# byungsook/deep-fluids

Hardware: AMD Instinct MI355X
Metric: velocity-field voxels/sec (3D 64x96x64 train step), whole job; per-GPU in `per_gpu` (higher is better)
Workload: dtype f32; 1 GPU; cfg3: 3D smoke3 64x96x64 (Z,Y,X) fp32, GeneratorBE3 filters=128 num_conv=4, per-GPU batch 16, full train step (fwd+curl3+jacobian3+L1 losses+bwd+Adam); global_batch=16, batch_per_gpu=16, params=7483523, parallelism=dp1

## Files before the change

### deep_fluids_amd/csrc/conv_wgrad.hip

```cpp
#include "df_common.hpp"

namespace {

using df::ceil_div;
typedef float f32x16 __attribute__((ext_vector_type(16)));
typedef float f32x2 __attribute__((ext_vector_type(2)));
typedef float f32x4 __attribute__((ext_vector_type(4)));

constexpr int kThreads = 256;
constexpr int kMaxRanges = 256;
constexpr int kZeroBytes = 512;
inline int64_t zero_row_bytes(int64_t W, int64_t Cin, int64_t Cout) {
  const int64_t Wp = ceil_div(W, 8) * 8 + 8;
  return Wp * (Cin > 2 * Cout ? Cin : 2 * Cout) * 4 + 64;
}
constexpr int kSmallStreams = 2048;

#ifdef DF_TUNING
int g_wgrad_dbg = 0;
#endif

struct WgradArgs {
  const float* x;
  const float* g;
// ... 1094 lines not shown
#pragma unroll
  for (int i = 0; i < 6; ++i) load_pos(cur, i, i);
  xc[0] = xcomb(0);

  auto tile = [&](int u, int x, const Row& lr, int lpos) {
    __builtin_amdgcn_sched_barrier(0);
    xc[(u + 1) & 7] = xcomb((u + 1) & 7);
    xc[(u + 2) & 7] = xcomb((u + 2) & 7);
    const f32x2 g0 = gcomb(u), g1 = gcomb((u + 1) & 7);
    f32x2 dm = xc[(u + 7) & 7], d0 = xc[u], d1 = xc[(u + 1) & 7], d2 = xc[(u + 2) & 7];
    if (x == 0) dm = f32x2{0.f, 0.f};
    if (x == Wc - 2) d2 = f32x2{0.f, 0.f};
    const f32x2 v0 = (DBG & 4) ? dm : wpk_sub(dm, d1), v1 = (DBG & 4) ? d0 : wpk_add(d0, d1), v2 = (DBG & 4) ? d1 : wpk_sub(d1, d0),
                v3 = (DBG & 4) ? d2 : wpk_sub(d0, d2);
    const f32x2 m1 = (DBG & 4) ? g0 : wpk_add(g0, g1), m2 = (DBG & 4) ? g1 : wpk_sub(g0, g1);
    if (!(DBG & 4)) bsum = wpk_add(bsum, m1);
    __builtin_amdgcn_sched_barrier(0);
    load_pos(lr, (u + 6) & 7, lpos);
    load_pos(lr, (u + 7) & 7, lpos + 1);
    if (UP) {
#pragma unroll
      for (int q = 0; q < 4; ++q) xr[q >> 1][q & 1][(u + 7) & 7] = xr[q >> 1][q & 1][(u + 6) & 7];
    }
    __builtin_amdgcn_sched_barrier(0);
#pragma unroll
    for (int s = 0; s < 2; ++s)
#pragma unroll
      for (int t = 0; t < 2; ++t) {
        acc[0][s][t] = __builtin_amdgcn_mfma_f32_32x32x2f32(v0[s], g0[t], acc[0][s][t], 0, 0, 0);
        acc[1][s][t] = __builtin_amdgcn_mfma_f32_32x32x2f32(v1[s], m1[t], acc[1][s][t], 0, 0, 0);
        if (!UP) acc[2][s][t] = __builtin_amdgcn_mfma_f32_32x32x2f32(v2[s], m2[t], acc[2][s][t], 0, 0, 0);
        acc[3][s][t] = __builtin_amdgcn_mfma_f32_32x32x2f32(v3[s], g1[t], acc[3][s][t], 0, 0, 0);
      }
  };

  for (int pair = p0; pair < p1; pair += pstep) {
    const Row nxt = row_setup(pair + pstep);
#pragma unroll
    for (int x0 = 0; x0 < Wc - 8; x0 += 8) {
#pragma unroll
      for (int u = 0; u < 8; u += 2) tile(u, x0 + u, cur, x0 + u + 6);
    }
    {
      constexpr int x0 = Wc - 8;
      tile(0, x0, cur, x0 + 6);
#pragma unroll
      for (int u = 2; u < 8; u += 2) tile(u, x0 + u, nxt, u - 2);
    }
    cur = nxt;
  }

  if constexpr (CS == 64) {
    float (*sR)[64 * 64] = reinterpret_cast<float (*)[64 * 64]>(lds);
    float (*sBs)[64] = reinterpret_cast<float (*)[64]>(lds + 4 * 64 * 64);
    float* P1 = a.partial + static_cast<int64_t>(range) * 64 * a.Cinp * a.Coutp;
#pragma unroll
    for (int d = 0; d < 4; ++d) {
      if (UP && d == 2) continue;
      const int slot = zy * 4 + d;
#pragma unroll
      for (int s = 0; s < 2; ++s)
#pragma unroll
        for (int t = 0; t < 2; ++t)
#pragma unroll
          for (int e = 0; e < 16; ++e) {
            const int i = (e & 3) + 8 * (e >> 2) + 4 * half;
            sR[sub][(2 * i + s) * 64 + 2 * r + t] = acc[d][s][t][e];
          }
      __syncthreads();
#pragma unroll
      for (int q = 0; q < 16; ++q) {
        const int j = q * kThreads + tid;
        const float v = ((sR[0][j] + sR[1][j]) + sR[2][j]) + sR[3][j];
        P1[(static_cast<int64_t>(slot) * a.Cinp + ci0 + (j >> 6)) * a.Coutp + co0 + (j & 63)] = v;
      }
      __syncthreads();
    }
    if (a.want_bias && GZ && GY && sel == 0 && blockIdx.y == 0) {
      bsum[0] += __shfl_xor(bsum[0], 32, 64);
      bsum[1] += __shfl_xor(bsum[1], 32, 64);
      if (half == 0) { sBs[sub][2 * r] = bsum[0]; sBs[sub][2 * r + 1] = bsum[1]; }
      __syncthreads();
      if (tid < 64) a.bpartial[static_cast<int64_t>(range) * a.Coutp + co0 + tid] = ((sBs[0][tid] + sBs[1][tid]) + sBs[2][tid]) + sBs[3][tid];
    }
    return;
  }
  float* P = a.partial + static_cast<int64_t>(erange) * 64 * a.Cinp * a.Coutp;
#pragma unroll
  for (int d = 0; d < 4; ++d) {
    if (UP && d == 2) continue;
    const int slot = zy * 4 + d;
#pragma unroll
    for (int s = 0; s < 2; ++s)
#pragma unroll
      for (int t = 0; t < 2; ++t)
#pragma unroll
        for (int e = 0; e < 16; ++e) {
          const int i = (e & 3) + 8 * (e >> 2) + 4 * half;
          const int ci = ci0 + 2 * i + s, co = co0 + 2 * r + t;
          P[(static_cast<int64_t>(slot) * a.Cinp + ci) * a.Coutp + co] = acc[d][s][t][e];
        }
  }
  if (do_bias) {
    bsum[0] += __shfl_xor(bsum[0], 32, 64);
    bsum[1] += __shfl_xor(bsum[1], 32, 64);
    if (half == 0) {
      float* pb = a.bpartial + static_cast<int64_t>(erange) * a.Coutp + co0 + 2 * r;
      pb[0] = bsum[0]; pb[1] = bsum[1];
    }
  }
}

template <int WP8, int CS, bool GZ, bool GY, bool UP = false, int DBG = 0>
__global__ __launch_bounds__(kThreads, 1) void wgrad_wxyz_kernel(const WxyzArgs aa) {
  constexpr int NT = ((UP && GZ) ? 1 : 2) * ((UP && GY) ? 1 : 2);
  __shared__ float sLds[CS == 64 ? kWxyzLds : 1];
  const int wg = wxyz_wg(aa.w.nranges * NT);
  wgrad_wxyz_body<WP8, CS, GZ, GY, UP, DBG>(aa, wg / NT, wg % NT, sLds);
}

template <int WP8, int CS, int DBG = 0>
__global__ __launch_bounds__(kThreads, 1) void wgrad_wxyz_fused_kernel(const WxyzArgs aa) {
  const int wg = wxyz_wg(aa.w.nranges * 16);
  const int range = wg >> 4, type = wg & 15;
  const int xiz = type >> 2, xiy = type & 3;
  const bool gz = xiz == 1 || xiz == 2, gy = xiy == 1 || xiy == 2;
  const int sel = (gz ? xiz - 1 : xiz / 3) * 2 + (gy ? xiy - 1 : xiy / 3);
  __shared__ float sLds[CS == 64 ? kWxyzLds : 1];
  if (gz && gy) wgrad_wxyz_body<WP8, CS, true, true, false, DBG>(aa, range, sel, sLds);
  else if (gz) wgrad_wxyz_body<WP8, CS, true, false, false, DBG>(aa, range, sel, sLds);
  else if (gy) wgrad_wxyz_body<WP8, CS, false, true, false, DBG>(aa, range, sel, sLds);
  else wgrad_wxyz_body<WP8, CS, false, false, false, DBG>(aa, range, sel, sLds);
}

template <int WP8, int CS>
__global__ __launch_bounds__(kThreads, 1) void wgrad_wxyz_up_fused_kernel(const WxyzArgs aa) {
  const int wg = wxyz_wg(aa.w.nranges * 9);
  const int range = wg / 9, t9 = wg % 9;
  const int zi = t9 / 3, yi = t9 % 3;
  const bool gz = zi == 1, gy = yi == 1;
  const int selz = zi == 2 ? 1 : 0, sely = yi == 2 ? 1 : 0;
  __shared__ float sLds[CS == 64 ? kWxyzLds : 1];
  if (gz && gy) wgrad_wxyz_body<WP8, CS, true, true, true, 0>(aa, range, 0, sLds);
  else if (gz) wgrad_wxyz_body<WP8, CS, true, false, true, 0>(aa, range, sely, sLds);
  else if (gy) wgrad_wxyz_body<WP8, CS, false, true, true, 0>(aa, range, selz, sLds);
  else wgrad_wxyz_body<WP8, CS, false, false, true, 0>(aa, range, selz * 2 + sely, sLds);
}

constexpr int kStgPos = 2 * 256;
template <int WP8> struct WxyzStage {
  static constexpr int Wc = WP8 * 8, NU = Wc / 4, BI = NU / 4, L = BI + 2;
  static constexpr int kLdsBytes = Wc * kStgPos * 4;
  static_assert(L >= BI + 1 && L <= NU - BI && L + 2 <= NU, "staging ring: write lead outside the barrier window");
  static_assert(kLdsBytes <= 160 * 1024, "staged (x,y,z) weight gradient: LDS image above gfx950's 160 KB");
};
static_assert(kWxyzLds * 4 <= 160 * 1024, "64-channel (x,y,z) weight gradient: LDS above gfx950's 160 KB");

template <int WP8, bool GZ, bool GY>
__device__ __forceinline__ void wgrad_wxyz_staged_body(const WxyzArgs& aa, int range, int sel, float* lds) {
  using ST = WxyzStage<WP8>;
  constexpr int Wc = ST::Wc, NU = ST::NU, BI = ST::BI, L = ST::L;
  const WgradArgs& a = aa.w;
  const int tid = threadIdx.x;
  const int lane = tid & 63;
  const int wave = __builtin_amdgcn_readfirstlane(tid >> 6);
  const int qi = wave >> 1, qj = wave & 1;
  const int half = lane >> 5, r = lane & 31;

  const int xiz = GZ ? 1 + sel / 2 : 3 * (sel / 2);
  const int xiy = GY ? 1 + sel % 2 : 3 * (sel % 2);
  const int zy = xiz * 4 + xiy;
  const int ci0 = qi * 64, co0 = qj * 64;
  const int p0 = range * a.pairs_per_range;
  int p1 = (range + 1) * a.pairs_per_range;
  if (p1 > a.npairs) p1 = a.npairs;

  const float* zb = a.zeros;
  const int yoa = xiy == 0 ? -1 : xiy == 2 ? 1 : 0, yob = xiy == 0 ? 1 : xiy == 1 ? 1 : xiy == 2 ? 0 : 2;
  const int zoa = xiz == 0 ? -1 : xiz == 2 ? 1 : 0, zob = xiz == 0 ? 1 : xiz == 1 ? 1 : xiz == 2 ? 0 : 2;
  const float syf = xiy == 1 ? 1.f : -1.f, szf = xiz == 1 ? 1.f : -1.f;
  const int gya = xiy == 3 ? 1 : 0, gza = xiz == 3 ? 1 : 0;
  const f32x2 sy2 = {syf, syf}, sz2 = {szf, szf};
  const int soff = wave * 128 + 4 * r;
  struct Row { const float* x[2][2]; const float* g[2][2]; };
  auto row_setup = [&](int pair) -> Row {
    Row rw;
    const int trow = 2 * pair + half;
    const bool ok = pair < p1 && trow < aa.ntrows;
    const int yt = trow % aa.Ht;
    const int t = trow / aa.Ht;
    const int zt = t % aa.Dt;
    const int b = t / aa.Dt;
    const int z0 = 2 * zt, y0 = 2 * yt;
    const int64_t bbase = static_cast<int64_t>(b) * a.D;
#pragma unroll
    for (int pz = 0; pz < 2; ++pz) {
      const int zs = z0 + (pz ? zob : zoa);
      const bool zv = ok && zs >= 0 && zs < a.D;
#pragma unroll
      for (int py = 0; py < 2; ++py) {
        const int ys = y0 + (py ? yob : yoa);
        rw.x[pz][py] = (zv && ys >= 0 && ys < a.H) ? a.x + ((bbase + zs) * a.H + ys) * Wc * 128 + soff : zb;
      }
      const int gz = z0 + (pz ? 1 : gza);
#pragma unroll
      for (int py = 0; py < 2; ++py) {
        const int gy = y0 + (py ? 1 : gya);
        const bool need = (pz == 0 || GZ) && (py == 0 || GY);
        rw.g[pz][py] = (need && ok) ? a.g + ((bbase + gz) * a.H + gy) * Wc * 128 + soff : zb;
      }
    }
    return rw;
  };
  auto ld4 = [&](const float* base, int unit) -> f32x4 { return *reinterpret_cast<const f32x4*>(base + unit * (4 * 128)); };
  auto pkfma = [&](f32x2 x, f32x2 y, f32x2 z) -> f32x2 {
    f32x2 d;
    asm("v_pk_fma_f32 %0, %1, %2, %3" : "=v"(d) : "v"(x), "v"(y), "v"(z));
    return d;
  };
  auto fma4 = [&](f32x4 x, f32x2 s, f32x4 z) -> f32x4 {
    const f32x2 lo = pkfma(f32x2{x[0], x[1]}, s, f32x2{z[0], z[1]}), hi = pkfma(f32x2{x[2], x[3]}, s, f32x2{z[2], z[3]});
    return f32x4{lo[0], lo[1], hi[0], hi[1]};
  };

  f32x16 acc[4][2][2];
#pragma unroll
  for (int d = 0; d < 4; ++d)
#pragma unroll
    for (int s = 0; s < 2; ++s)
#pragma unroll
      for (int t = 0; t < 2; ++t)
#pragma unroll
        for (int e = 0; e < 16; ++e) acc[d][s][t][e] = 0.f;
  f32x2 bsum = {0.f, 0.f};
  const bool do_bias = a.want_bias && GZ && GY && sel == 0 && qi == 0;

  f32x4 sx[2][2][2], sg[2][2][2];
  float* const wst = lds + wave * kStgPos + half * 256 + 4 * r;
  const float* const rdx = lds + half * 256 + ci0 + 2 * r;
  const float* const rdg = lds + half * 256 + 128 + co0 + 2 * r;
  auto load_x = [&](const Row& lr, int set, int unit) {
#pragma unroll
    for (int q = 0; q < 4; ++q) sx[set][q >> 1][q & 1] = ld4(lr.x[q >> 1][q & 1], unit);
  };
  auto load_g = [&](const Row& lr, int set, int unit) {
    sg[set][0][0] = ld4(lr.g[0][0], unit);
    if (GY) sg[set][0][1] = ld4(lr.g[0][1], unit);
    if (GZ) sg[set][1][0] = ld4(lr.g[1][0], unit);
    if (GZ && GY) sg[set][1][1] = ld4(lr.g[1][1], unit);
  };
  auto store_x = [&](int set, int unit) {
    const f32x4 ta = fma4(sx[set][0][1], sy2, sx[set][0][0]), tb = fma4(sx[set][1][1], sy2, sx[set][1][0]);
    *reinterpret_cast<f32x4*>(wst + unit * (4 * kStgPos)) = fma4(tb, sz2, ta);
  };
  auto store_g = [&](int set, int unit) {
    f32x4 v;
    if (GZ && GY) {
      const f32x4 ta = fma4(sg[set][0][1], sy2, sg[set][0][0]), tb = fma4(sg[set][1][1], sy2, sg[set][1][0]);
      v = fma4(tb, sz2, ta);
    } else if (GY) v = fma4(sg[set][0][1], sy2, sg[set][0][0]);
    else if (GZ) v = fma4(sg[set][1][0], sz2, sg[set][0][0]);
    else v = sg[set][0][0];
    *reinterpret_cast<f32x4*>(wst + unit * (4 * kStgPos) + 128) = v;
  };
  auto lds_sync = [&]() { asm volatile("s_waitcnt lgkmcnt(0)\n\ts_barrier" ::: "memory"); };

  f32x2 xq[8], gq[4];
  auto rd_x = [&](int pos) { xq[pos & 7] = *reinterpret_cast<const f32x2*>(rdx + (pos % Wc) * kStgPos); };
  auto rd_g = [&](int pos) { gq[pos & 3] = *reinterpret_cast<const f32x2*>(rdg + (pos % Wc) * kStgPos); };

  Row cur = row_setup(p0);
#pragma unroll
  for (int u = 0; u < L; ++u) {
    load_x(cur, u & 1, u); load_g(cur, u & 1, u);
    store_x(u & 1, u); store_g(u & 1, u);
  }
#pragma unroll
  for (int u = L; u < L + 2; ++u) { load_x(cur, u & 1, u); load_g(cur, u & 1, u); }
  lds_sync();
  rd_x(0); rd_x(1); rd_x(2); rd_g(0); rd_g(1);
  xq[7] = f32x2{0.f, 0.f};

  auto step = [&](int u, const Row& lc, const Row& ln) {
    const int x = 2 * u, k = u >> 1;
    __builtin_amdgcn_sched_barrier(0);
    const f32x2 g0 = gq[x & 3], g1 = gq[(x + 1) & 3];
    f32x2 dm = xq[(x + 7) & 7], d0 = xq[x & 7], d1 = xq[(x + 1) & 7], d2 = xq[(x + 2) & 7];
    if (x == 0) dm = f32x2{0.f, 0.f};
    if (x == Wc - 2) d2 = f32x2{0.f, 0.f};
    const f32x2 v0 = wpk_sub(dm, d1), v1 = wpk_add(d0, d1), v2 = wpk_sub(d1, d0), v3 = wpk_sub(d0, d2);
    const f32x2 m1 = wpk_add(g0, g1), m2 = wpk_sub(g0, g1);
    bsum = wpk_add(bsum, m1);
    __builtin_amdgcn_sched_barrier(0);
    rd_x(x + 3); rd_x(x + 4); rd_g(x + 2); rd_g(x + 3);
    {
      const int m = k + L, set = m & 1;
      if ((u & 1) == 0) {
        store_x(set, m % NU);
        load_x(m + 2 < NU ? lc : ln, set, (m + 2) % NU);
      } else {
        store_g(set, m % NU);
        load_g(m + 2 < NU ? lc : ln, set, (m + 2) % NU);
      }
    }
    __builtin_amdgcn_sched_barrier(0);
#pragma unroll
    for (int s = 0; s < 2; ++s)
#pragma unroll
      for (int t = 0; t < 2; ++t) {
        acc[0][s][t] = __builtin_amdgcn_mfma_f32_32x32x2f32(v0[s], g0[t], acc[0][s][t], 0, 0, 0);
        acc[1][s][t] = __builtin_amdgcn_mfma_f32_32x32x2f32(v1[s], m1[t], acc[1][s][t], 0, 0, 0);
        acc[2][s][t] = __builtin_amdgcn_mfma_f32_32x32x2f32(v2[s], m2[t], acc[2][s][t], 0, 0, 0);
        acc[3][s][t] = __builtin_amdgcn_mfma_f32_32x32x2f32(v3[s], g1[t], acc[3][s][t], 0, 0, 0);
      }
    if ((u & 1) && (k + 1) % BI == 0) lds_sync();
  };

  for (int pair = p0; pair < p1; ++pair) {
    const Row nxt = row_setup(pair + 1);
#pragma unroll
    for (int u = 0; u < Wc / 2; ++u) step(u, cur, nxt);
    cur = nxt;
  }

  float* P = a.partial + static_cast<int64_t>(range) * 64 * a.Cinp * a.Coutp;
#pragma unroll
  for (int d = 0; d < 4; ++d) {
    const int slot = zy * 4 + d;
#pragma unroll
    for (int s = 0; s < 2; ++s)
#pragma unroll
      for (int t = 0; t < 2; ++t)
#pragma unroll
        for (int e = 0; e < 16; ++e) {
          const int i = (e & 3) + 8 * (e >> 2) + 4 * half;
          const int ci = ci0 + 2 * i + s, co = co0 + 2 * r + t;
          P[(static_cast<int64_t>(slot) * a.Cinp + ci) * a.Coutp + co] = acc[d][s][t][e];
        }
  }
  if (do_bias) {
    bsum[0] += __shfl_xor(bsum[0], 32, 64);
    bsum[1] += __shfl_xor(bsum[1], 32, 64);
    if (half == 0) {
      float* pb = a.bpartial + static_cast<int64_t>(range) * a.Coutp + co0 + 2 * r;
      pb[0] = bsum[0]; pb[1] = bsum[1];
    }
  }
}

template <int WP8>
__global__ __launch_bounds__(kThreads, 1) void wgrad_wxyz_staged_kernel(const WxyzArgs aa) {
  const int wg = wxyz_wg(aa.w.nranges * 16);
  const int range = wg >> 4, type = wg & 15;
  const int xiz = type >> 2, xiy = type & 3;
  const bool gz = xiz == 1 || xiz == 2, gy = xiy == 1 || xiy == 2;
  const int sel = (gz ? xiz - 1 : xiz / 3) * 2 + (gy ? xiy - 1 : xiy / 3);
  __shared__ __attribute__((aligned(16))) float sStage[WxyzStage<WP8>::kLdsBytes / 4];
  if (gz && gy) wgrad_wxyz_staged_body<WP8, true, true>(aa, range, sel, sStage);
  else if (gz) wgrad_wxyz_staged_body<WP8, true, false>(aa, range, sel, sStage);
  else if (gy) wgrad_wxyz_staged_body<WP8, false, true>(aa, range, sel, sStage);
  else wgrad_wxyz_staged_body<WP8, false, false>(aa, range, sel, sStage);
}

__global__ __launch_bounds__(kThreads) void wgrad_wxyz_reduce_kernel(const float* __restrict__ partial, const float* __restrict__ bpartial,
                                                                     float* __restrict__ gw, float* __restrict__ gb, int nranges, int Cin,
                                                                     int Cout, int Cinp, int Coutp, int up) {
  __shared__ float sV[8][27][32];
  const int64_t total = static_cast<int64_t>(Cin) * Cout;
  const int64_t slot = static_cast<int64_t>(Cinp) * Coutp;
  const int64_t pstride = 64 * slot;
  const int el = threadIdx.x & 31, grp = threadIdx.x >> 5;
  const int64_t i = static_cast<int64_t>(blockIdx.x) * 32 + el;
  const bool ok = i < total;
  const int co = ok ? static_cast<int>(i % Cout) : 0;
  const int ci = ok ? static_cast<int>(i / Cout) : 0;
  const float* p = partial + static_cast<int64_t>(ci) * Coutp + co;
  float u[64];
#pragma unroll
  for (int k = 0; k < 64; ++k) u[k] = 0.f;
  if (ok) {
    for (int rg = grp; rg < nranges; rg += 8) {
      const float* q = p + rg * pstride;
#pragma unroll
      for (int k = 0; k < 64; ++k)
        if (!(up && ((k >> 4) == 2 || ((k >> 2) & 3) == 2 || (k & 3) == 2))) u[k] += q[k * slot];
    }
  }
  float a1[16][3];
#pragma unroll
  for (int k = 0; k < 16; ++k) {
    const float h = 0.5f * (u[k * 4 + 1] + u[k * 4 + 2]);
    a1[k][0] = u[k * 4] + h; a1[k][1] = 0.5f * (u[k * 4 + 1] - u[k * 4 + 2]); a1[k][2] = h - u[k * 4 + 3];
  }
  float a2[4][3][3];
#pragma unroll
  for (int z = 0; z < 4; ++z)
#pragma unroll
    for (int dx = 0; dx < 3; ++dx) {
      const float h = 0.5f * (a1[z * 4 + 1][dx] + a1[z * 4 + 2][dx]);
      a2[z][0][dx] = a1[z * 4][dx] + h; a2[z][1][dx] = 0.5f * (a1[z * 4 + 1][dx] - a1[z * 4 + 2][dx]); a2[z][2][dx] = h - a1[z * 4 + 3][dx];
    }
#pragma unroll
  for (int dy = 0; dy < 3; ++dy)
#pragma unroll
    for (int dx = 0; dx < 3; ++dx) {
      const float h = 0.5f * (a2[1][dy][dx] + a2[2][dy][dx]);
      sV[grp][0 * 9 + dy * 3 + dx][el] = a2[0][dy][dx] + h;
      sV[grp][1 * 9 + dy * 3 + dx][el] = 0.5f * (a2[1][dy][dx] - a2[2][dy][dx]);
      sV[grp][2 * 9 + dy * 3 + dx][el] = h - a2[3][dy][dx];
    }
  __syncthreads();
  for (int k = grp; k < 27; k += 8) {
    if (!ok) break;
    float t = sV[0][k][el];
#pragma unroll
    for (int g = 1; g < 8; ++g) t += sV[g][k][el];
    gw[(static_cast<int64_t>(k) * Cin + ci) * Cout + co] = t;
  }
  if (gb && static_cast<int>(blockIdx.x) * 32 < Cout) bias_reduce_cols(bpartial, gb, nranges, Cout, Coutp, &sV[0][0][0], blockIdx.x);
}

inline bool wx_ok(int64_t W, int64_t Cin, int64_t Cout) {
  return (W == 16 || W == 32 || W == 64 || W == 56 || W == 112 || W == 128 || W == 96 || W == 48) && Cin % 2 == 0 && Cout % 2 == 0 && Cin >= 32 && Cout >= 32;
}
inline bool wxy_ok(int64_t H, int64_t W, int64_t Cin, int64_t Cout) { return wx_ok(W, Cin, Cout) && H % 2 == 0 && H >= 4; }
inline bool wxyz_ok(int64_t D, int64_t H, int64_t W, int64_t Cin, int64_t Cout, int kz) {
  if (!(kz == 3 && wxy_ok(H, W, Cin, Cout) && D % 2 == 0 && D >= 4)) return false;
  if (Cin == 128 && Cout == 128) return W == 64 || W == 32 || W == 16 || W == 112 || W == 56 || W == 128;
  if (Cin == 64 && Cout == 64) return W == 128 || W == 64 || W == 32 || W == 16;
  return false;
}
inline int wgrad_algo(int req, int64_t rows, int64_t D, int64_t H, int64_t W, int64_t Cin, int64_t Cout, int kz) {
  if (req == 1) return 0;
  if ((req == 0 || req == 4) && wxyz_ok(D, H, W, Cin, Cout, kz)) return 3;
  if (req != 2 && wxy_ok(H, W, Cin, Cout) && (rows >= 4096 || req >= 3)) return 2;
  return wx_ok(W, Cin, Cout) ? 1 : 0;
}

typedef __bf16 bf16x8 __attribute__((ext_vector_type(8)));

__device__ __forceinline__ void split8(const float (&x)[8], bf16x8& hi, bf16x8& lo) {
#pragma unroll
  for (int e = 0; e < 8; ++e) {
    const __bf16 h = static_cast<__bf16>(x[e]);
    hi[e] = h;
    lo[e] = static_cast<__bf16>(x[e] - static_cast<float>(h));
  }
}

constexpr int cgcd(int a, int b) { return b == 0 ? a : cgcd(b, a % b); }

template <int W16>
__global__ __launch_bounds__(kThreads, 1) void wgrad_bf16x3_kernel(const WgradArgs a) {
  constexpr int U = 4 / cgcd(W16, 4);
  constexpr int NS = U * W16;
  constexpr int E = (3 + W16 - 1) / W16;
  const int tid = threadIdx.x;
  const int lane = tid & 63;
  const int wave = __builtin_amdgcn_readfirstlane(tid >> 6);
  const int nq = a.nqi * a.nqj;
  const int qi = (wave % nq) / a.nqj, qj = (wave % nq) % a.nqj, sub = wave / nq;
  const int half = lane >> 5, r = lane & 31;

  const int nwg = a.nranges * a.ndzdy;
  int wg;
  {
    const int bid = blockIdx.x, q = nwg >> 3, rem = nwg & 7;
    const int xcd = bid & 7, idx = bid >> 3;
    wg = (xcd < rem ? xcd * (q + 1) : rem * (q + 1) + (xcd - rem) * q) + idx;
  }
  const int range = wg / a.ndzdy, dzdy = wg % a.ndzdy;
  int dz, dy, pz = 0, py = 0, px = 0, dd = 0, cls = 0;
  if (a.up) {
    const int nd2 = a.ndzdy == 32 ? 4 : 2;
    cls = dzdy / nd2; dd = dzdy % nd2;
    pz = a.ndzdy == 32 ? (cls >> 2) & 1 : 0; py = (cls >> 1) & 1; px = cls & 1;
    dz = a.ndzdy == 32 ? (dd >> 1) + pz - 1 : 0;
    dy = (dd & 1) + py - 1;
  } else {
    dz = a.ndzdy == 9 ? dzdy / 3 - 1 : 0;
    dy = (a.ndzdy == 9 ? dzdy % 3 : dzdy) - 1;
  }
  const int gs = a.up ? 2 : 1;
  const int ci0 = blockIdx.y * 128 + qi * 64, co0 = blockIdx.z * 128 + qj * 64;
  if (ci0 >= a.Cin || co0 >= a.Cout) return;

  const int ppe = (a.pairs_per_range + a.nsub - 1) / a.nsub;
  const int row0 = 2 * (range * a.pairs_per_range + sub * ppe);
  int row1 = row0 + 2 * ppe;
  if (row1 > 2 * (range + 1) * a.pairs_per_range) row1 = 2 * (range + 1) * a.pairs_per_range;
  if (row1 > a.nrows) row1 = a.nrows;
  const int erange = range * a.nsub + sub;
  const int cia = ci0 + 2 * r, coa = co0 + 2 * r;
  const bool ci_ok = cia < a.Cin, co_ok = coa < a.Cout;
  const float* zb = a.zeros;

  struct Row { const float* xb; const float* gb; bool xz; };
  auto row_setup = [&](int row) -> Row {
    Row rw;
    const bool ok = row < row1;
    const int y = row % a.H;
    const int t = row / a.H;
    const int z = t % a.D;
    const int b = t / a.D;
    const int zs = z + dz, ys = y + dy;
    const bool xv = ok && zs >= 0 && zs < a.D && ys >= 0 && ys < a.H && ci_ok;
    const bool gv = ok && co_ok;
    const int64_t gvox = ((static_cast<int64_t>(b) * a.gD + (z * gs + pz)) * a.gH + (y * gs + py)) * a.gW + px;
    const int64_t xvox = ((static_cast<int64_t>(b) * a.D + zs) * a.H + ys) * a.W;
    rw.xb = xv ? a.x + (xvox + 8 * half) * a.Cin + cia : zb;
    rw.gb = gv ? a.g + (gvox + 8 * half * gs) * a.Cout + coa : zb;
    rw.xz = !xv;
    return rw;
  };
// ... 869 lines not shown
    else if (W == 96) DF_WXY(12, 0);
    else if (W == 48 && c128) DF_WXY(6, 128);
    else if (W == 48) DF_WXY(6, 0);
    else if (W == 112) DF_WXY(14, 0);
    else if (W == 56) DF_WXY(7, 0);
    else if (W == 32 && c128) DF_WXY(4, 128);
    else if (W == 32) DF_WXY(4, 0);
    else if (c128) DF_WXY(2, 128);
    else DF_WXY(2, 0);
#undef DF_WXY
    const int ndz = kz == 3 ? 3 : 1;
    const int64_t tot = static_cast<int64_t>(ndz) * Cin * Cout;
    const int64_t rgx = ceil_div(tot, 32);
    hipLaunchKernelGGL(wgrad_wxy_reduce_kernel, dim3((unsigned)rgx), dim3(kThreads), 0, s, a.partial, a.bpartial, gw, gb,
                       p.nranges * p.nsub, ndz, (int)Cin, (int)Cout, p.Cinp, p.Coutp);
    return df::launched("df_conv_wgrad(winograd-xy)");
  } else if (algo == 1) {
    const bool c128 = Cin == 128 && Cout == 128;
    if (W == 64 && c128) hipLaunchKernelGGL((wgrad_wx_kernel<8, 128>), grid, dim3(kThreads), 0, s, a);
    else if (W == 64) hipLaunchKernelGGL((wgrad_wx_kernel<8, 0>), grid, dim3(kThreads), 0, s, a);
    else if (W == 128) hipLaunchKernelGGL((wgrad_wx_kernel<16, 0>), grid, dim3(kThreads), 0, s, a);
    else if (W == 96) hipLaunchKernelGGL((wgrad_wx_kernel<12, 0>), grid, dim3(kThreads), 0, s, a);
    else if (W == 48) hipLaunchKernelGGL((wgrad_wx_kernel<6, 0>), grid, dim3(kThreads), 0, s, a);
    else if (W == 112) hipLaunchKernelGGL((wgrad_wx_kernel<14, 0>), grid, dim3(kThreads), 0, s, a);
    else if (W == 56) hipLaunchKernelGGL((wgrad_wx_kernel<7, 0>), grid, dim3(kThreads), 0, s, a);
    else if (W == 32 && c128) hipLaunchKernelGGL((wgrad_wx_kernel<4, 128>), grid, dim3(kThreads), 0, s, a);
    else if (W == 32) hipLaunchKernelGGL((wgrad_wx_kernel<4, 0>), grid, dim3(kThreads), 0, s, a);
    else if (c128) hipLaunchKernelGGL((wgrad_wx_kernel<2, 128>), grid, dim3(kThreads), 0, s, a);
    else hipLaunchKernelGGL((wgrad_wx_kernel<2, 0>), grid, dim3(kThreads), 0, s, a);
    const int64_t tot = static_cast<int64_t>(p.ndzdy) * Cin * Cout;
    const int64_t rgx = ceil_div(tot, 32) + (gb ? ceil_div(Cout, 32) : 0);
    hipLaunchKernelGGL(wgrad_wx_reduce_kernel, dim3((unsigned)rgx), dim3(kThreads), 0, s, a.partial, a.bpartial, gw, gb,
                       p.nranges * p.nsub, p.ndzdy, (int)Cin, (int)Cout, p.Cinp, p.Coutp);
    return df::launched("df_conv_wgrad(winograd-x)");
  } else {
  const int wp8 = a.Wp / 8;
  const bool exact = (W % 8) == 0;
  if (xvec && gvec && exact && wp8 == 8) hipLaunchKernelGGL((wgrad_kernel<true, true, 8>), grid, dim3(kThreads), 0, s, a);
  else if (xvec && gvec && exact && wp8 == 16) hipLaunchKernelGGL((wgrad_kernel<true, true, 16>), grid, dim3(kThreads), 0, s, a);
  else if (xvec && gvec && exact && wp8 == 4) hipLaunchKernelGGL((wgrad_kernel<true, true, 4>), grid, dim3(kThreads), 0, s, a);
  else if (xvec && gvec && exact && wp8 == 14) hipLaunchKernelGGL((wgrad_kernel<true, true, 14>), grid, dim3(kThreads), 0, s, a);
  else if (xvec && gvec && exact && wp8 == 12) hipLaunchKernelGGL((wgrad_kernel<true, true, 12>), grid, dim3(kThreads), 0, s, a);
  else if (xvec && gvec && exact && wp8 == 7) hipLaunchKernelGGL((wgrad_kernel<true, true, 7>), grid, dim3(kThreads), 0, s, a);
  else if (xvec && gvec && exact && wp8 == 2) hipLaunchKernelGGL((wgrad_kernel<true, true, 2>), grid, dim3(kThreads), 0, s, a);
  else if (xvec && gvec && exact && wp8 == 3) hipLaunchKernelGGL((wgrad_kernel<true, true, 3>), grid, dim3(kThreads), 0, s, a);
  else if (xvec && gvec && exact && wp8 == 6) hipLaunchKernelGGL((wgrad_kernel<true, true, 6>), grid, dim3(kThreads), 0, s, a);
  else if (xvec && gvec) hipLaunchKernelGGL((wgrad_kernel<true, true, 0>), grid, dim3(kThreads), 0, s, a);
  else if (xvec) hipLaunchKernelGGL((wgrad_kernel<true, false, 0>), grid, dim3(kThreads), 0, s, a);
  else if (gvec) hipLaunchKernelGGL((wgrad_kernel<false, true, 0>), grid, dim3(kThreads), 0, s, a);
  else hipLaunchKernelGGL((wgrad_kernel<false, false, 0>), grid, dim3(kThreads), 0, s, a);
  }
  const int64_t total = static_cast<int64_t>(p.taps) * Cin * Cout;
  const int64_t rg = ceil_div(total, 32) + (gb ? ceil_div(Cout, 32) : 0);
  hipLaunchKernelGGL(wgrad_reduce_kernel, dim3((unsigned)rg), dim3(kThreads), 0, s, a.partial, a.bpartial, gw, gb,
                     p.nranges * p.nsub, p.taps, (int)Cin, (int)Cout, p.Cinp, p.Coutp);
  return df::launched("df_conv_wgrad");
}

int df_conv_wgrad(const float* x, const float* gy, float* gw, float* gb, int64_t B, int64_t D, int64_t H, int64_t W,
                  int64_t Cin, int64_t Cout, int kz, void* workspace, int64_t workspace_bytes, df_stream_t stream) {
  return conv_wgrad_impl(x, gy, gw, gb, B, D, H, W, Cin, Cout, kz, workspace, workspace_bytes, stream, 0, 0);
}
int df_conv_wgrad_algo(const float* x, const float* gy, float* gw, float* gb, int64_t B, int64_t D, int64_t H, int64_t W,
                       int64_t Cin, int64_t Cout, int kz, void* workspace, int64_t workspace_bytes, int algo, df_stream_t stream) {
  return conv_wgrad_impl(x, gy, gw, gb, B, D, H, W, Cin, Cout, kz, workspace, workspace_bytes, stream, 0, algo);
}
int df_conv_wgrad_bf16x3(const float* x, const float* gy, float* gw, float* gb, int64_t B, int64_t D, int64_t H, int64_t W,
                         int64_t Cin, int64_t Cout, int kz, void* workspace, int64_t workspace_bytes, df_stream_t stream) {
  return conv_wgrad_impl(x, gy, gw, gb, B, D, H, W, Cin, Cout, kz, workspace, workspace_bytes, stream, 1, 0);
}

static bool s2_wgrad_ok(int64_t Wo, int64_t Cin, int64_t Cout) {
  return (Wo == 8 || Wo == 16 || Wo == 32 || Wo == 64) && Cin % 2 == 0 && Cout % 2 == 0 && Cin >= 32 && Cout >= 32;
}
int64_t df_conv_s2_wgrad_workspace_bytes(int64_t B, int64_t Do, int64_t Ho, int64_t Wo, int64_t Cin, int64_t Cout, int kz) {
  if (B <= 0 || Do <= 0 || Ho <= 0 || Wo <= 0 || Cin <= 0 || Cout <= 0 || !s2_wgrad_ok(Wo, Cin, Cout)) return 0;
  const Plan p = make_plan(B, Do, Ho, Wo, Cin, Cout, kz);
  return (p.partial_elems + p.bpartial_elems) * static_cast<int64_t>(sizeof(float)) + zero_row_bytes(2 * Wo, Cin, Cout);
}
int df_conv_s2_wgrad(const float* x, const float* gy, float* gw, float* gb, int64_t B, int64_t Do, int64_t Ho, int64_t Wo, int64_t Cin,
                     int64_t Cout, int kz, void* workspace, int64_t workspace_bytes, df_stream_t stream) {
  DF_REQUIRE(x && gy && gw && workspace, DF_EINVAL, "df_conv_s2_wgrad: null pointer");
  DF_REQUIRE(B > 0 && Do > 0 && Ho > 0 && Wo > 0 && Cin > 0 && Cout > 0, DF_EINVAL, "df_conv_s2_wgrad: non-positive extent");
  DF_REQUIRE(kz == 1 || kz == 3, DF_ESHAPE, "df_conv_s2_wgrad: kz must be 1 (2-D) or 3 (3-D)");
  DF_REQUIRE(kz == 3 || Do == 1, DF_ESHAPE, "df_conv_s2_wgrad: Do must be 1 when kz == 1");
  DF_REQUIRE(s2_wgrad_ok(Wo, Cin, Cout), DF_ESHAPE,
             "df_conv_s2_wgrad: output rows of 8 | 16 | 32 | 64 voxels and even channel counts >= 32 only (other shapes: df_dilate2_odd + df_conv_wgrad)");
  DF_REQUIRE(B * Do * Ho < (1LL << 30) && 8 * B * Do * Ho * Wo * Cin < (1LL << 40), DF_ESHAPE, "df_conv_s2_wgrad: tensor too large");
  DF_REQUIRE(df::aligned16(workspace) && (reinterpret_cast<uintptr_t>(x) & 7u) == 0 && (reinterpret_cast<uintptr_t>(gy) & 7u) == 0, DF_EALIGN,
             "df_conv_s2_wgrad: workspace must be 16-byte, x and gy 8-byte aligned");
  DF_REQUIRE(workspace_bytes >= df_conv_s2_wgrad_workspace_bytes(B, Do, Ho, Wo, Cin, Cout, kz), DF_EWORKSPACE, "df_conv_s2_wgrad: workspace too small");
  const Plan p = make_plan(B, Do, Ho, Wo, Cin, Cout, kz);
  WgradArgs a;
  a.x = x; a.g = gy;
  a.partial = static_cast<float*>(workspace);
  a.bpartial = a.partial + p.partial_elems;
  float* zeros = a.bpartial + p.bpartial_elems;
  a.zeros = zeros;
  a.B = (int)B; a.D = (int)Do; a.H = (int)Ho; a.W = (int)Wo; a.Cin = (int)Cin; a.Cout = (int)Cout;
  a.Cinp = p.Cinp; a.Coutp = p.Coutp;
  a.Wp = (int)Wo;
  a.nrows = p.nrows; a.npairs = p.npairs; a.nranges = p.nranges; a.pairs_per_range = p.ppr;
  a.ndzdy = p.ndzdy; a.want_bias = gb != nullptr;
  a.nqi = p.nqi; a.nqj = p.nqj; a.nsub = p.nsub;
  a.up = 0; a.gD = a.D; a.gH = a.H; a.gW = a.W;
  hipStream_t s = df::as_stream(stream);
  if (hipError_t e = df::zero_async(zeros, zero_row_bytes(2 * Wo, Cin, Cout), s)) return df::fail((int)e, "df_conv_s2_wgrad: memset: %s", hipGetErrorString(e));
  dim3 grid((unsigned)(p.nranges * p.ndzdy), (unsigned)ceil_div(Cin, 128), (unsigned)ceil_div(Cout, 128));
  if (Wo == 64) hipLaunchKernelGGL((wgrad_s2_kernel<8>), grid, dim3(kThreads), 0, s, a);
  else if (Wo == 32) hipLaunchKernelGGL((wgrad_s2_kernel<4>), grid, dim3(kThreads), 0, s, a);
  else if (Wo == 16) hipLaunchKernelGGL((wgrad_s2_kernel<2>), grid, dim3(kThreads), 0, s, a);
  else hipLaunchKernelGGL((wgrad_s2_kernel<1>), grid, dim3(kThreads), 0, s, a);
  const int64_t total = static_cast<int64_t>(p.taps) * Cin * Cout;
  const int64_t rg = ceil_div(total, 32) + (gb ? ceil_div(Cout, 32) : 0);
  hipLaunchKernelGGL(wgrad_reduce_kernel, dim3((unsigned)rg), dim3(kThreads), 0, s, a.partial, a.bpartial, gw, gb,
                     p.nranges * p.nsub, p.taps, (int)Cin, (int)Cout, p.Cinp, p.Coutp);
  return df::launched("df_conv_s2_wgrad");
}

int df_conv_wgrad_form(int64_t B, int64_t D, int64_t H, int64_t W, int64_t Cin, int64_t Cout, int kz, int algo) {
  if (B <= 0 || D <= 0 || H <= 0 || W <= 0 || Cin <= 0 || Cout <= 0 || (kz != 1 && kz != 3) || algo < 0 || (algo & 7) > 4) return DF_EINVAL;
  const int req = algo & 7;
  const bool swap = Cin <= 4 && Cout >= 64;
  const int64_t Cw = swap ? Cout : Cin, Ct = swap ? Cin : Cout;
  if ((swap || small_n_ok(Cin, Cout)) && req != 1 && thin_mfma_ok(B, D, H, W, Cw, Ct, kz) && thin_mfma_inst(W, Cw, Ct, swap)) return 10;
  if (small_n_ok(Cin, Cout)) return 11;
  if (Cin % 2 || Cout % 2) return 0;
  if (wxyz_padded_w(req, D, H, W, Cin, Cout, kz)) return 3;
  return wgrad_algo(req, B * D * H, D, H, W, Cin, Cout, kz);
}

static Plan make_up_plan(int64_t B, int64_t Dc, int64_t Hc, int64_t Wc, int64_t Cin, int64_t Cout, int kz) {
  Plan p = make_plan(B, Dc, Hc, Wc, Cin, Cout, kz);
  p.ndzdy = kz == 3 ? 32 : 8;
  const int nr = p.npairs >= 64 ? 64 : p.npairs;
  p.ppr = (p.npairs + nr - 1) / nr;
  p.nranges = (p.npairs + p.ppr - 1) / p.ppr;
  p.taps = p.ndzdy * 3;
  p.partial_elems = static_cast<int64_t>(p.nranges) * p.nsub * p.taps * p.Cinp * p.Coutp;
  p.bpartial_elems = static_cast<int64_t>(p.nranges) * p.nsub * (kz == 3 ? 8 : 4) * p.Coutp;
  return p;
}

static bool up_wxyz_ok(int req, int64_t B, int64_t Dc, int64_t Hc, int64_t Wc, int64_t Cin, int64_t Cout, int kz) {
  (void)B;
  return wxyz_ok(2 * Dc, 2 * Hc, 2 * Wc, Cin, Cout, kz) && req != 1 && req != 2 && req != 3;
}

static int up_wxyz_ranges(int64_t B, int64_t Dc, int64_t Hc, int64_t Cin = 128, int64_t Cout = 128) {
  return ((B * Dc * Hc + 1) / 2 < 4096 || (Cin <= 64 && Cout <= 64)) ? 28 : 113;
}

int df_upconv_wgrad_form(int64_t B, int64_t Dc, int64_t Hc, int64_t Wc, int64_t Cin, int64_t Cout, int kz, int algo) {
  if (B <= 0 || Dc <= 0 || Hc <= 0 || Wc <= 0 || Cin <= 0 || Cout <= 0 || (kz != 1 && kz != 3) || algo < 0 || algo > 4) return DF_EINVAL;
  return up_wxyz_ok(algo, B, Dc, Hc, Wc, Cin, Cout, kz) ? 3 : 0;
}

int64_t df_upconv_wgrad_workspace_bytes(int64_t B, int64_t Dc, int64_t Hc, int64_t Wc, int64_t Cin, int64_t Cout, int kz) {
  if (B <= 0 || Dc <= 0 || Hc <= 0 || Wc <= 0 || Cin <= 0 || Cout <= 0) return 0;
  if (wxyz_ok(2 * Dc, 2 * Hc, 2 * Wc, Cin, Cout, kz)) {
    const Plan q = make_plan(B, 2 * Dc, 2 * Hc, 2 * Wc, Cin, Cout, kz, 3, up_wxyz_ranges(B, Dc, Hc, Cin, Cout));
    const Plan p = make_up_plan(B, Dc, Hc, Wc, Cin, Cout, kz);
    const int64_t nq = (q.partial_elems + q.bpartial_elems) * static_cast<int64_t>(sizeof(float)) + zero_row_bytes(2 * Wc, Cin, Cout);
    const int64_t np = (p.partial_elems + p.bpartial_elems) * static_cast<int64_t>(sizeof(float)) + zero_row_bytes(Wc, Cin, Cout);
    return nq > np ? nq : np;
  }
  const Plan p = make_up_plan(B, Dc, Hc, Wc, Cin, Cout, kz);
  return (p.partial_elems + p.bpartial_elems) * static_cast<int64_t>(sizeof(float)) + zero_row_bytes(Wc, Cin, Cout);
}

static int upconv_wgrad_impl(const float* xc, const float* gy, float* gw, float* gb, int64_t B, int64_t Dc, int64_t Hc,
                             int64_t Wc, int64_t Cin, int64_t Cout, int kz, void* workspace, int64_t workspace_bytes,
                             df_stream_t stream, int prec, int req) {
  DF_REQUIRE(req >= 0 && req <= 4, DF_EINVAL, "df_upconv_wgrad: algo must be 0..4");
  DF_REQUIRE(xc && gy && gw && workspace, DF_EINVAL, "df_upconv_wgrad: null pointer");
  DF_REQUIRE(B > 0 && Dc > 0 && Hc > 0 && Wc > 0 && Cin > 0 && Cout > 0, DF_EINVAL, "df_upconv_wgrad: non-positive extent");
  DF_REQUIRE(kz == 1 || kz == 3, DF_ESHAPE, "df_upconv_wgrad: kz must be 1 (2-D) or 3 (3-D)");
  DF_REQUIRE(kz == 3 || Dc == 1, DF_ESHAPE, "df_upconv_wgrad: Dc must be 1 when kz == 1");
  DF_REQUIRE(Cin % 2 == 0 && Cout % 2 == 0, DF_ESHAPE, "df_upconv_wgrad: even channel counts only");
  DF_REQUIRE(df::aligned16(workspace), DF_EALIGN, "df_upconv_wgrad: workspace must be 16-byte aligned");
  DF_REQUIRE(workspace_bytes >= df_upconv_wgrad_workspace_bytes(B, Dc, Hc, Wc, Cin, Cout, kz), DF_EWORKSPACE,
             "df_upconv_wgrad: workspace too small");
  if (up_wxyz_ok(req, B, Dc, Hc, Wc, Cin, Cout, kz) && df::aligned16(xc) && df::aligned16(gy)) {
    const int64_t D = 2 * Dc, H = 2 * Hc, W = 2 * Wc;
    const Plan p = make_plan(B, D, H, W, Cin, Cout, kz, 3, up_wxyz_ranges(B, Dc, Hc, Cin, Cout));
    WxyzArgs aa;
    WgradArgs& a = aa.w;
    a.x = xc; a.g = gy;
    a.partial = static_cast<float*>(workspace);
    a.bpartial = a.partial + p.partial_elems;
    float* zeros = a.bpartial + p.bpartial_elems;
    a.zeros = zeros;
    a.B = (int)B; a.D = (int)D; a.H = (int)H; a.W = (int)W; a.Cin = (int)Cin; a.Cout = (int)Cout;
    a.Cinp = p.Cinp; a.Coutp = p.Coutp;
    a.Wp = (int)W;
    a.nrows = p.nrows; a.npairs = p.npairs; a.nranges = p.nranges; a.pairs_per_range = p.ppr;
    a.ndzdy = p.ndzdy; a.want_bias = gb != nullptr;
    a.nqi = p.nqi; a.nqj = p.nqj; a.nsub = p.nsub;
    a.up = 0; a.gD = a.D; a.gH = a.H; a.gW = a.W;
    aa.Ht = (int)Hc; aa.Dt = (int)Dc; aa.ntrows = p.nrows;
    hipStream_t s = df::as_stream(stream);
    if (hipError_t e = df::zero_async(zeros, zero_row_bytes(W, Cin, Cout), s)) return df::fail((int)e, "df_upconv_wgrad: memset: %s", hipGetErrorString(e));
    const unsigned gy_ = (unsigned)ceil_div(Cin, 128), gz_ = (unsigned)ceil_div(Cout, 128);
    const dim3 gridu((unsigned)(p.nranges * 9), gy_, gz_);
#define DF_UWXYZ(WP) hipLaunchKernelGGL((wgrad_wxyz_up_fused_kernel<WP, 128>), gridu, dim3(kThreads), 0, s, aa)
#define DF_UWXYZ64(WP) hipLaunchKernelGGL((wgrad_wxyz_up_fused_kernel<WP, 64>), gridu, dim3(kThreads), 0, s, aa)
    if (Cin == 64) { if (W == 128) DF_UWXYZ64(16); else if (W == 64) DF_UWXYZ64(8); else if (W == 32) DF_UWXYZ64(4); else DF_UWXYZ64(2); }
    else
    if (W == 64) DF_UWXYZ(8); else if (W == 32) DF_UWXYZ(4); else if (W == 16) DF_UWXYZ(2); else if (W == 112) DF_UWXYZ(14); else if (W == 128) DF_UWXYZ(16); else DF_UWXYZ(7);
#undef DF_UWXYZ
#undef DF_UWXYZ64
    const int64_t rgx = ceil_div(Cin * Cout, 32);
    hipLaunchKernelGGL(wgrad_wxyz_reduce_kernel, dim3((unsigned)rgx), dim3(kThreads), 0, s, a.partial, a.bpartial, gw, gb,
                       Cin == 64 ? p.nranges : p.nranges * p.nsub, (int)Cin, (int)Cout, p.Cinp, p.Coutp, 1);
    return df::launched("df_upconv_wgrad(winograd-xyz, 27-point)");
  }
  const Plan p = make_up_plan(B, Dc, Hc, Wc, Cin, Cout, kz);
  WgradArgs a;
  a.x = xc; a.g = gy;
  a.partial = static_cast<float*>(workspace);
  a.bpartial = a.partial + p.partial_elems;
  float* zeros = a.bpartial + p.bpartial_elems;
  a.zeros = zeros;
  a.B = (int)B; a.D = (int)Dc; a.H = (int)Hc; a.W = (int)Wc; a.Cin = (int)Cin; a.Cout = (int)Cout;
  a.Cinp = p.Cinp; a.Coutp = p.Coutp;
  a.Wp = (int)(ceil_div(Wc, 8) * 8);
  a.nrows = p.nrows; a.npairs = p.npairs; a.nranges = p.nranges; a.pairs_per_range = p.ppr;
  a.ndzdy = p.ndzdy; a.want_bias = gb != nullptr;
  a.nqi = p.nqi; a.nqj = p.nqj; a.nsub = p.nsub;
  a.up = 1; a.gD = kz == 3 ? 2 * a.D : 1; a.gH = 2 * a.H; a.gW = 2 * a.W;
  hipStream_t s = df::as_stream(stream);
  if (hipError_t e = df::zero_async(zeros, zero_row_bytes(Wc, Cin, Cout), s)) return df::fail((int)e, "df_upconv_wgrad: memset: %s", hipGetErrorString(e));
  dim3 grid((unsigned)(p.nranges * p.ndzdy), (unsigned)ceil_div(Cin, 128), (unsigned)ceil_div(Cout, 128));
  const int wp8 = a.Wp / 8;
  const bool exact = (Wc % 8) == 0;
  const bool aligned8 = ((reinterpret_cast<uintptr_t>(xc) | reinterpret_cast<uintptr_t>(gy)) & 7u) == 0;
  const dim3 grid2((unsigned)(p.nranges * (p.ndzdy / 2)), grid.y, grid.z);
  if (prec == 1 && wgrad_bf16x3_ok(Wc, Cin, Cout)) launch_wgrad_bf16x3(Wc, grid, s, a);
  else if (aligned8 && exact && wp8 == 4 && Cin == 128 && Cout == 128 && req != 1) hipLaunchKernelGGL((wgrad_up2_kernel<4, 128>), grid2, dim3(kThreads), 0, s, a);
  else if (aligned8 && exact && wp8 == 6 && Cin == 128 && Cout == 128 && req != 1) hipLaunchKernelGGL((wgrad_up2_kernel<6, 128>), grid2, dim3(kThreads), 0, s, a);
  else if (aligned8 && exact && wp8 == 3 && Cin == 128 && Cout == 128 && req != 1) hipLaunchKernelGGL((wgrad_up2_kernel<3, 128>), grid2, dim3(kThreads), 0, s, a);
  else if (aligned8 && exact && wp8 == 2 && req != 1) hipLaunchKernelGGL((wgrad_up2_kernel<2, 0>), grid2, dim3(kThreads), 0, s, a);
  else if (aligned8 && exact && wp8 == 1 && req != 1) hipLaunchKernelGGL((wgrad_up2_kernel<1, 0>), grid2, dim3(kThreads), 0, s, a);
  else if (exact && wp8 == 8) hipLaunchKernelGGL((wgrad_kernel<true, true, 8>), grid, dim3(kThreads), 0, s, a);
  else if (exact && wp8 == 4) hipLaunchKernelGGL((wgrad_kernel<true, true, 4>), grid, dim3(kThreads), 0, s, a);
  else if (exact && wp8 == 2) hipLaunchKernelGGL((wgrad_kernel<true, true, 2>), grid, dim3(kThreads), 0, s, a);
  else if (exact && wp8 == 7) hipLaunchKernelGGL((wgrad_kernel<true, true, 7>), grid, dim3(kThreads), 0, s, a);
  else hipLaunchKernelGGL((wgrad_kernel<true, true, 0>), grid, dim3(kThreads), 0, s, a);
  const int64_t total = static_cast<int64_t>(kz * 9) * Cin * Cout;
  const int64_t rg = ceil_div(total, 32);
  hipLaunchKernelGGL(wgrad_up_reduce_kernel, dim3((unsigned)rg), dim3(kThreads), 0, s, a.partial, a.bpartial, gw, gb,
                     p.nranges * p.nsub, kz, (int)Cin, (int)Cout, p.Cinp, p.Coutp);
  return df::launched("df_upconv_wgrad");
}

int df_upconv_wgrad(const float* xc, const float* gy, float* gw, float* gb, int64_t B, int64_t Dc, int64_t Hc, int64_t Wc,
                    int64_t Cin, int64_t Cout, int kz, void* workspace, int64_t workspace_bytes, df_stream_t stream) {
  return upconv_wgrad_impl(xc, gy, gw, gb, B, Dc, Hc, Wc, Cin, Cout, kz, workspace, workspace_bytes, stream, 0, 0);
}
int df_upconv_wgrad_algo(const float* xc, const float* gy, float* gw, float* gb, int64_t B, int64_t Dc, int64_t Hc, int64_t Wc,
                         int64_t Cin, int64_t Cout, int kz, void* workspace, int64_t workspace_bytes, int algo, df_stream_t stream) {
  return upconv_wgrad_impl(xc, gy, gw, gb, B, Dc, Hc, Wc, Cin, Cout, kz, workspace, workspace_bytes, stream, 0, algo);
}
int df_upconv_wgrad_bf16x3(const float* xc, const float* gy, float* gw, float* gb, int64_t B, int64_t Dc, int64_t Hc,
                           int64_t Wc, int64_t Cin, int64_t Cout, int kz, void* workspace, int64_t workspace_bytes,
                           df_stream_t stream) {
  return upconv_wgrad_impl(xc, gy, gw, gb, B, Dc, Hc, Wc, Cin, Cout, kz, workspace, workspace_bytes, stream, 1, 0);
}

}
```

Baseline: 36.77 million voxels/s.

## Add staged LDS-ring up-sampling weight-gradient kernel for 128-channel W=64

Adds an UP variant of the LDS-staged (x,y,z) Winograd weight-gradient body. It reads the coarse pre-upsample input directly at half resolution, stages one x column per two output positions, and drops the acc[2] MFMA term, which is zero for nearest-upsampled input. The new kernel is dispatched by default for Cin=Cout=128 at W=64, replacing the fused up kernel. The aim is to cut global loads, LDS traffic and MFMA work in the upconv weight gradient. The cost is more complex ring indexing with new static_assert constraints.

```diff
diff --git a/deep_fluids_amd/csrc/conv_wgrad.hip b/deep_fluids_amd/csrc/conv_wgrad.hip
--- a/deep_fluids_amd/csrc/conv_wgrad.hip
+++ b/deep_fluids_amd/csrc/conv_wgrad.hip
@@ -1270,11 +1270,12 @@
   static constexpr int Wc = WP8 * 8, NU = Wc / 4, BI = NU / 4, L = BI + 2;
   static constexpr int kLdsBytes = Wc * kStgPos * 4;
   static_assert(L >= BI + 1 && L <= NU - BI && L + 2 <= NU, "staging ring: write lead outside the barrier window");
+  static_assert(L % 2 == 0 && L + 1 <= NU - BI && L + 4 <= NU, "staging ring (up-sampling form): write lead outside the barrier window");
   static_assert(kLdsBytes <= 160 * 1024, "staged (x,y,z) weight gradient: LDS image above gfx950's 160 KB");
 };
 static_assert(kWxyzLds * 4 <= 160 * 1024, "64-channel (x,y,z) weight gradient: LDS above gfx950's 160 KB");
 
-template <int WP8, bool GZ, bool GY>
+template <int WP8, bool GZ, bool GY, bool UP = false>
 __device__ __forceinline__ void wgrad_wxyz_staged_body(const WxyzArgs& aa, int range, int sel, float* lds) {
   using ST = WxyzStage<WP8>;
   constexpr int Wc = ST::Wc, NU = ST::NU, BI = ST::BI, L = ST::L;
@@ -1285,8 +1286,9 @@
   const int qi = wave >> 1, qj = wave & 1;
   const int half = lane >> 5, r = lane & 31;
 
-  const int xiz = GZ ? 1 + sel / 2 : 3 * (sel / 2);
-  const int xiy = GY ? 1 + sel % 2 : 3 * (sel % 2);
+  constexpr int NTY = (UP && GY) ? 1 : 2;
+  const int xiz = GZ ? 1 + sel / NTY : 3 * (sel / NTY);
+  const int xiy = GY ? 1 + sel % NTY : 3 * (sel % NTY);
   const int zy = xiz * 4 + xiy;
   const int ci0 = qi * 64, co0 = qj * 64;
   const int p0 = range * a.pairs_per_range;
@@ -1318,7 +1320,9 @@
 #pragma unroll
       for (int py = 0; py < 2; ++py) {
         const int ys = y0 + (py ? yob : yoa);
-        rw.x[pz][py] = (zv && ys >= 0 && ys < a.H) ? a.x + ((bbase + zs) * a.H + ys) * Wc * 128 + soff : zb;
+        if (UP) rw.x[pz][py] = (zv && ys >= 0 && ys < a.H)
+                                   ? a.x + ((static_cast<int64_t>(b) * (a.D >> 1) + (zs >> 1)) * (a.H >> 1) + (ys >> 1)) * (Wc / 2) * 128 + soff : zb;
+        else rw.x[pz][py] = (zv && ys >= 0 && ys < a.H) ? a.x + ((bbase + zs) * a.H + ys) * Wc * 128 + soff : zb;
       }
       const int gz = z0 + (pz ? 1 : gza);
 #pragma unroll
@@ -1355,6 +1359,7 @@
 
   f32x4 sx[2][2][2], sg[2][2][2];
   float* const wst = lds + wave * kStgPos + half * 256 + 4 * r;
+  float* const wstx = UP ? lds + 2 * wave * kStgPos + half * 256 + 4 * r : wst;
   const float* const rdx = lds + half * 256 + ci0 + 2 * r;
   const float* const rdg = lds + half * 256 + 128 + co0 + 2 * r;
   auto load_x = [&](const Row& lr, int set, int unit) {
@@ -1369,7 +1374,7 @@
   };
   auto store_x = [&](int set, int unit) {
     const f32x4 ta = fma4(sx[set][0][1], sy2, sx[set][0][0]), tb = fma4(sx[set][1][1], sy2, sx[set][1][0]);
-    *reinterpret_cast<f32x4*>(wst + unit * (4 * kStgPos)) = fma4(tb, sz2, ta);
+    *reinterpret_cast<f32x4*>(wstx + unit * (4 * kStgPos)) = fma4(tb, sz2, ta);
   };
   auto store_g = [&](int set, int unit) {
     f32x4 v;
@@ -1385,35 +1390,53 @@
 
   f32x2 xq[8], gq[4];
   auto rd_x = [&](int pos) { xq[pos & 7] = *reinterpret_cast<const f32x2*>(rdx + (pos % Wc) * kStgPos); };
+  auto rd_xc = [&](int cpos) { xq[cpos & 3] = *reinterpret_cast<const f32x2*>(rdx + ((2 * cpos) % Wc) * kStgPos); };
   auto rd_g = [&](int pos) { gq[pos & 3] = *reinterpret_cast<const f32x2*>(rdg + (pos % Wc) * kStgPos); };
 
   Row cur = row_setup(p0);
 #pragma unroll
   for (int u = 0; u < L; ++u) {
-    load_x(cur, u & 1, u); load_g(cur, u & 1, u);
-    store_x(u & 1, u); store_g(u & 1, u);
-  }
-#pragma unroll
-  for (int u = L; u < L + 2; ++u) { load_x(cur, u & 1, u); load_g(cur, u & 1, u); }
+    if (!UP) load_x(cur, u & 1, u);
+    else if ((u & 1) == 0) load_x(cur, (u >> 1) & 1, u >> 1);
+    load_g(cur, u & 1, u);
+    if (!UP) store_x(u & 1, u);
+    else if ((u & 1) == 0) store_x((u >> 1) & 1, u);
+    store_g(u & 1, u);
+  }
+#pragma unroll
+  for (int u = L; u < L + 2; ++u) {
+    if (!UP) load_x(cur, u & 1, u);
+    else { const int j = (L >> 1) + (u - L); load_x(cur, j & 1, j); }
+    load_g(cur, u & 1, u);
+  }
   lds_sync();
-  rd_x(0); rd_x(1); rd_x(2); rd_g(0); rd_g(1);
-  xq[7] = f32x2{0.f, 0.f};
+  if (UP) { rd_xc(0); rd_xc(1); xq[3] = f32x2{0.f, 0.f}; }
+  else { rd_x(0); rd_x(1); rd_x(2); xq[7] = f32x2{0.f, 0.f}; }
+  rd_g(0); rd_g(1);
 
   auto step = [&](int u, const Row& lc, const Row& ln) {
     const int x = 2 * u, k = u >> 1;
     __builtin_amdgcn_sched_barrier(0);
     const f32x2 g0 = gq[x & 3], g1 = gq[(x + 1) & 3];
-    f32x2 dm = xq[(x + 7) & 7], d0 = xq[x & 7], d1 = xq[(x + 1) & 7], d2 = xq[(x + 2) & 7];
+    f32x2 dm = xq[UP ? (u + 3) & 3 : (x + 7) & 7], d0 = xq[UP ? u & 3 : x & 7], d1 = xq[UP ? u & 3 : (x + 1) & 7],
+          d2 = xq[UP ? (u + 1) & 3 : (x + 2) & 7];
     if (x == 0) dm = f32x2{0.f, 0.f};
     if (x == Wc - 2) d2 = f32x2{0.f, 0.f};
     const f32x2 v0 = wpk_sub(dm, d1), v1 = wpk_add(d0, d1), v2 = wpk_sub(d1, d0), v3 = wpk_sub(d0, d2);
     const f32x2 m1 = wpk_add(g0, g1), m2 = wpk_sub(g0, g1);
     bsum = wpk_add(bsum, m1);
     __builtin_amdgcn_sched_barrier(0);
-    rd_x(x + 3); rd_x(x + 4); rd_g(x + 2); rd_g(x + 3);
+    if (UP) rd_xc(u + 2);
+    else { rd_x(x + 3); rd_x(x + 4); }
+    rd_g(x + 2); rd_g(x + 3);
     {
       const int m = k + L, set = m & 1;
-      if ((u & 1) == 0) {
+      if (UP && (u & 1) == 0) {
+        if ((u & 3) == 0) {
+          store_x((m >> 1) & 1, m % NU);
+          load_x(m + 4 < NU ? lc : ln, (m >> 1) & 1, ((m + 4) % NU) >> 1);
+        }
+      } else if ((u & 1) == 0) {
         store_x(set, m % NU);
         load_x(m + 2 < NU ? lc : ln, set, (m + 2) % NU);
       } else {
@@ -1428,7 +1451,7 @@
       for (int t = 0; t < 2; ++t) {
         acc[0][s][t] = __builtin_amdgcn_mfma_f32_32x32x2f32(v0[s], g0[t], acc[0][s][t], 0, 0, 0);
         acc[1][s][t] = __builtin_amdgcn_mfma_f32_32x32x2f32(v1[s], m1[t], acc[1][s][t], 0, 0, 0);
-        acc[2][s][t] = __builtin_amdgcn_mfma_f32_32x32x2f32(v2[s], m2[t], acc[2][s][t], 0, 0, 0);
+        if (!UP) acc[2][s][t] = __builtin_amdgcn_mfma_f32_32x32x2f32(v2[s], m2[t], acc[2][s][t], 0, 0, 0);
         acc[3][s][t] = __builtin_amdgcn_mfma_f32_32x32x2f32(v3[s], g1[t], acc[3][s][t], 0, 0, 0);
       }
     if ((u & 1) && (k + 1) % BI == 0) lds_sync();
@@ -1444,6 +1467,7 @@
   float* P = a.partial + static_cast<int64_t>(range) * 64 * a.Cinp * a.Coutp;
 #pragma unroll
   for (int d = 0; d < 4; ++d) {
+    if (UP && d == 2) continue;
     const int slot = zy * 4 + d;
 #pragma unroll
     for (int s = 0; s < 2; ++s)
@@ -1478,6 +1502,20 @@
   else if (gz) wgrad_wxyz_staged_body<WP8, true, false>(aa, range, sel, sStage);
   else if (gy) wgrad_wxyz_staged_body<WP8, false, true>(aa, range, sel, sStage);
   else wgrad_wxyz_staged_body<WP8, false, false>(aa, range, sel, sStage);
+}
+
+template <int WP8>
+__global__ __launch_bounds__(kThreads, 1) void wgrad_wxyz_up_staged_kernel(const WxyzArgs aa) {
+  const int wg = wxyz_wg(aa.w.nranges * 9);
+  const int range = wg / 9, t9 = wg % 9;
+  const int zi = t9 / 3, yi = t9 % 3;
+  const bool gz = zi == 1, gy = yi == 1;
+  const int selz = zi == 2 ? 1 : 0, sely = yi == 2 ? 1 : 0;
+  __shared__ __attribute__((aligned(16))) float sStage[WxyzStage<WP8>::kLdsBytes / 4];
+  if (gz && gy) wgrad_wxyz_staged_body<WP8, true, true, true>(aa, range, 0, sStage);
+  else if (gz) wgrad_wxyz_staged_body<WP8, true, false, true>(aa, range, sely, sStage);
+  else if (gy) wgrad_wxyz_staged_body<WP8, false, true, true>(aa, range, selz, sStage);
+  else wgrad_wxyz_staged_body<WP8, false, false, true>(aa, range, selz * 2 + sely, sStage);
 }
 
 __global__ __launch_bounds__(kThreads) void wgrad_wxyz_reduce_kernel(const float* __restrict__ partial, const float* __restrict__ bpartial,
@@ -2653,7 +2691,7 @@
 }
 
 int df_upconv_wgrad_form(int64_t B, int64_t Dc, int64_t Hc, int64_t Wc, int64_t Cin, int64_t Cout, int kz, int algo) {
-  if (B <= 0 || Dc <= 0 || Hc <= 0 || Wc <= 0 || Cin <= 0 || Cout <= 0 || (kz != 1 && kz != 3) || algo < 0 || algo > 4) return DF_EINVAL;
+  if (B <= 0 || Dc <= 0 || Hc <= 0 || Wc <= 0 || Cin <= 0 || Cout <= 0 || (kz != 1 && kz != 3) || algo < 0 || algo > 6) return DF_EINVAL;
   return up_wxyz_ok(algo, B, Dc, Hc, Wc, Cin, Cout, kz) ? 3 : 0;
 }
 
@@ -2673,7 +2711,7 @@
 static int upconv_wgrad_impl(const float* xc, const float* gy, float* gw, float* gb, int64_t B, int64_t Dc, int64_t Hc,
                              int64_t Wc, int64_t Cin, int64_t Cout, int kz, void* workspace, int64_t workspace_bytes,
                              df_stream_t stream, int prec, int req) {
-  DF_REQUIRE(req >= 0 && req <= 4, DF_EINVAL, "df_upconv_wgrad: algo must be 0..4");
+  DF_REQUIRE(req >= 0 && req <= 6, DF_EINVAL, "df_upconv_wgrad: algo must be 0..6");
   DF_REQUIRE(xc && gy && gw && workspace, DF_EINVAL, "df_upconv_wgrad: null pointer");
   DF_REQUIRE(B > 0 && Dc > 0 && Hc > 0 && Wc > 0 && Cin > 0 && Cout > 0, DF_EINVAL, "df_upconv_wgrad: non-positive extent");
   DF_REQUIRE(kz == 1 || kz == 3, DF_ESHAPE, "df_upconv_wgrad: kz must be 1 (2-D) or 3 (3-D)");
@@ -2706,6 +2744,9 @@
     const dim3 gridu((unsigned)(p.nranges * 9), gy_, gz_);
 #define DF_UWXYZ(WP) hipLaunchKernelGGL((wgrad_wxyz_up_fused_kernel<WP, 128>), gridu, dim3(kThreads), 0, s, aa)
 #define DF_UWXYZ64(WP) hipLaunchKernelGGL((wgrad_wxyz_up_fused_kernel<WP, 64>), gridu, dim3(kThreads), 0, s, aa)
+    if (req != 5 && Cin == 128 && Cout == 128 && W == 64) hipLaunchKernelGGL((wgrad_wxyz_up_staged_kernel<8>), gridu, dim3(kThreads), 0, s, aa);
+    else if (req == 6 && Cin == 128 && Cout == 128 && W == 32) hipLaunchKernelGGL((wgrad_wxyz_up_staged_kernel<4>), gridu, dim3(kThreads), 0, s, aa);
+    else
     if (Cin == 64) { if (W == 128) DF_UWXYZ64(16); else if (W == 64) DF_UWXYZ64(8); else if (W == 32) DF_UWXYZ64(4); else DF_UWXYZ64(2); }
     else
     if (W == 64) DF_UWXYZ(8); else if (W == 32) DF_UWXYZ(4); else if (W == 16) DF_UWXYZ(2); else if (W == 112) DF_UWXYZ(14); else if (W == 128) DF_UWXYZ(16); else DF_UWXYZ(7);
```

Measured after the change: 36.79 million voxels/s, median of 4. Within noise of the previous version (+0.1%).
